# XiangFeng-Wen/STF-Unet

Hardware: AMD Instinct MI355X
Metric: training samples/sec (256x256 DCE-MRI frames) (higher is better)
Workload: dtype bf16; 1 GPU; cfg2 UNet(in=8,base_c=64) 256x256 train step; model=UNet, global_batch=64, per_gpu_batch=64, seq_len=8, parallelism=dp1, ddp_hook=False

## Files before the change

### include/stfunet.h

```cpp
#ifndef STFUNET_H
#define STFUNET_H
#include <stddef.h>
#include <stdint.h>

#ifdef __cplusplus
extern "C" {
#endif

typedef void* stf_stream_t;

typedef struct stf_conv_geom {
  int N;
  int Hs, Ws, Cs;
  int src_cstride;
  int Hd, Wd;
  int R, S;
  int stride, pad;
  int transposed;
} stf_conv_geom;

typedef struct stf_lstm_epi {
  const float* c_prev;
  float* c_out;
  void* h_out;
// ... 210 lines not shown
int stf_resize_bilinear_fwd(const float* x, int planes, int h, int w, float* y, int H, int W, stf_stream_t stream);
int stf_resize_bilinear_bwd(const float* dy, int planes, int H, int W, float* dx, int h, int w, stf_stream_t stream);
int stf_lstm_unpack_grad(const float* dwcat, const float* dbias, int C, float* dw_ih,
                         float* dw_hh, float* db_ih, float* db_hh, stf_stream_t stream);
int stf_lstm_cell_bwd(const float* gates, const float* c_t, const float* c_prev, const void* dh,
                      int dh_cstride, const float* dc_in, float* dc_out, void* dgates, int64_t M,
                      int C, stf_stream_t stream);
int stf_pk_resize(const float* x, int B, int Ttot, int T, int P, int H, int W, int h, int w,
                  void* dst, int dst_cstride, int coff, stf_stream_t stream);

int stf_eval_counts(const float* logits, const int64_t* target, int B, int K, int64_t HW,
                    int64_t ignore_index, int64_t* confmat, int64_t* dice_counts, stf_stream_t stream);
int stf_eval_counts_sm(const float* logits, const float* probs, const int64_t* target, int B, int K,
                       int64_t HW, int64_t ignore_index, int64_t* confmat, int64_t* dice_counts,
                       stf_stream_t stream);

int stf_predict_mask(const float* logits, const int64_t* target, int B, int K, int64_t HW, int rule,
                     int channel, float threshold, int64_t ignore, uint8_t* mask, int64_t* counts,
                     stf_stream_t stream);
size_t stf_predict_overlay_scratch_bytes(int B, int64_t HW);
int stf_predict_overlay(const float* frames, int64_t batch_stride, const uint8_t* mask, int B, int H,
                        int W, int c0, int c1, int c2, float alpha, int paint, uint8_t* out,
                        void* scratch, stf_stream_t stream);

int stf_tofts_forward(const float* ktrans, const float* ve, const float* vp, int P, int T,
                      const float* time_points, const float* cp_t, const float* tau,
                      const float* cp_tau, const int* n_valid, int n_conv, float dt, float* out,
                      stf_stream_t stream);
int stf_tofts_fit(const float* curves, int P, int T, const float* time_points, const float* cp_t,
                  const float* tau, const float* cp_tau, const int* n_valid, int n_conv, float dt,
                  int batch, int epochs, const float* adam_sched, float beta1, float beta2, float eps,
                  const float* bounds, float* params, stf_stream_t stream);

#define STF_AUG_HFLIP 1
#define STF_AUG_VFLIP 2
#define STF_AUG_ROTATE 4
typedef struct stf_aug_frame {
  int64_t src, rs, out;
  int H, W, H2, W2;
  int cx, cy, kx, ky;
  int oh, ow, h0, w0;
  int flags;
  int fx[6];
  int pad_;
  double m[6];
} stf_aug_frame;
int stf_augment_frames(const uint8_t* src, const stf_aug_frame* frames, int n, const int* coef,
                       uint8_t* scratch, int max_resized_px, int max_out_px, float mean, float stdv,
                       float* out, stf_stream_t stream);
int stf_augment_masks(const uint8_t* src, const stf_aug_frame* masks, int n, const int* tabs,
                      int max_out_px, int64_t* out, stf_stream_t stream);

typedef struct stf_plan stf_plan;
stf_plan* stf_plan_create(void);
void stf_plan_destroy(stf_plan* plan);
int stf_plan_record(stf_plan* plan);
int stf_plan_stop(void);
int stf_plan_size(const stf_plan* plan);
int stf_plan_tag(const char* name, double flops);
int stf_plan_tag_end(void);
int stf_plan_replay(stf_plan* plan, int first, int last, const char* timed_tag);
int stf_plan_timing(stf_plan* plan, int* launches, double* ms, double* flops);
int stf_stream_wait(stf_stream_t waiter, stf_stream_t waitee);
int stf_memset(void* p, int value, size_t bytes, stf_stream_t stream);
int stf_copy_rows(const float* src, int64_t src_ld, float* dst, int64_t dst_ld, int rows, int cols,
                  stf_stream_t stream);
int stf_i64_add_batch(int64_t* const* ptrs, int count, int64_t inc, stf_stream_t stream);

const char* stf_error_string(int code);
int stf_abi_version(void);

#define STF_STORAGE_BF16 0
#define STF_STORAGE_FP16 1
int stf_storage_type(void);

#ifdef __cplusplus
}
#endif
#endif
```

### stf-unet_amd/csrc/common.h

```cpp
#pragma once
#include <hip/hip_runtime.h>
#include <stdint.h>

#include <tuple>
#include <type_traits>
#include <utility>

#ifdef STF_FP16
typedef _Float16 e16;
#else
typedef __bf16 e16;
#endif
typedef e16 e16x8 __attribute__((ext_vector_type(8)));
typedef e16 e16x4 __attribute__((ext_vector_type(4)));
typedef short short4v __attribute__((ext_vector_type(4)));
typedef float f32x4 __attribute__((ext_vector_type(4)));
typedef float f32x16 __attribute__((ext_vector_type(16)));
typedef unsigned int u32x4v __attribute__((ext_vector_type(4)));

#define STF_DEV __device__ __forceinline__

STF_DEV float e2f(e16 v) { return (float)v; }
STF_DEV e16 f2e(float v) { return (e16)v; }

// ... 55 lines not shown
  gi = sigm(pi); gf = sigm(pf); gg = tanh_f(pg); go = sigm(po);
  c = __builtin_fmaf(gf, cp, gi * gg);
  h = go * tanh_f(c);
}
STF_DEV void lstm_cell_bwd(float gi, float gf, float gg, float go, float ct, float cp, float dh, float dcn,
                           float& d_i, float& d_f, float& d_g, float& d_o, float& dcp) {
#pragma clang fp contract(off)
  const float tc = tanh_f(ct);
  const float dct = __builtin_fmaf(dh * go, __builtin_fmaf(-tc, tc, 1.f), dcn);
  d_o = ((dh * tc) * go) * (1.f - go);
  d_i = ((dct * gg) * gi) * (1.f - gi);
  d_g = (dct * gi) * __builtin_fmaf(-gg, gg, 1.f);
  d_f = ((dct * cp) * gf) * (1.f - gf);
  dcp = dct * gf;
}

STF_DEV float wave_sum(float v) {
#pragma unroll
  for (int o = 32; o > 0; o >>= 1) v += __shfl_xor(v, o, 64);
  return v;
}

template <int CTRL>
STF_DEV float dpp_f(float v) {
  return __int_as_float(__builtin_amdgcn_update_dpp(0, __float_as_int(v), CTRL, 0xF, 0xF, true));
}

STF_DEV float row16_reduce_scatter(const float (&v)[16], int r) {
  float a[8], b[4], c[2];
  const bool h3 = r & 8, h2 = r & 4, h1 = r & 2, h0 = r & 1;
#pragma unroll
  for (int k = 0; k < 8; ++k) a[k] = (h3 ? v[k + 8] : v[k]) + dpp_f<0x140>(h3 ? v[k] : v[k + 8]);
#pragma unroll
  for (int k = 0; k < 4; ++k) b[k] = (h2 ? a[k + 4] : a[k]) + dpp_f<0x141>(h2 ? a[k] : a[k + 4]);
#pragma unroll
  for (int k = 0; k < 2; ++k) c[k] = (h1 ? b[k + 2] : b[k]) + dpp_f<0x1B>(h1 ? b[k] : b[k + 2]);
  return (h0 ? c[1] : c[0]) + dpp_f<0xB1>(h0 ? c[0] : c[1]);
}

STF_DEV double wave_sum_d(double v) {
#pragma unroll
  for (int o = 32; o > 0; o >>= 1) v += __shfl_xor(v, o, 64);
  return v;
}

namespace stf {
struct PlanOp {
  virtual ~PlanOp() {}
  virtual hipError_t run() const = 0;
};
bool plan_recording();
void plan_append(PlanOp* op, hipStream_t s);

template <class... A>
struct KernelOp final : PlanOp {
  const void* fn;
  dim3 grid, block;
  unsigned shmem;
  hipStream_t stream;
  std::tuple<A...> args;
  template <class... B>
  KernelOp(const void* f, dim3 g, dim3 b, unsigned sh, hipStream_t s, B&&... a)
      : fn(f), grid(g), block(b), shmem(sh), stream(s), args(std::forward<B>(a)...) {}
  hipError_t run() const override {
    return std::apply(
        [this](const A&... a) {
          void* p[sizeof...(A) + 1] = {const_cast<void*>(static_cast<const void*>(&a))...};
          return hipLaunchKernel(fn, grid, block, p, shmem, stream);
        },
        args);
  }
};

template <class... A, class... B>
inline void launch(void (*k)(A...), dim3 g, dim3 b, unsigned sh, hipStream_t s, B&&... args) {
  static_assert(sizeof...(A) == sizeof...(B), "kernel argument count");
  if (!plan_recording()) {
    std::tuple<std::decay_t<A>...> t(std::forward<B>(args)...);
    std::apply(
        [&](auto&... a) {
          void* p[sizeof...(A) + 1] = {static_cast<void*>(&a)...};
          (void)hipLaunchKernel((const void*)k, g, b, p, sh, s);
        },
        t);
    return;
  }
  auto* op = new KernelOp<std::decay_t<A>...>((const void*)k, g, b, sh, s, std::forward<B>(args)...);
  (void)op->run();
  plan_append(op, s);
}

hipError_t memset_async(void* p, int value, size_t bytes, hipStream_t s);
int ablation_env(const char* name);
char ab_letter(const char* name);
hipError_t memcpy_async(void* dst, const void* src, size_t bytes, hipMemcpyKind kind, hipStream_t s);
}

#undef hipLaunchKernelGGL
#define hipLaunchKernelGGL(K, G, B, SH, S, ...) ::stf::launch(K, G, B, SH, S, ##__VA_ARGS__)

#define STF_CHECK_LAUNCH() do { hipError_t e__ = hipGetLastError(); if (e__ != hipSuccess) return (int)e__; } while (0)

#define STF_EINVAL 100001
```

### stf-unet_amd/csrc/loss.hip

```cpp
#include "common.h"
#include "../../include/stfunet.h"
#include "reduce.h"

namespace {

constexpr int NT = 256;
constexpr int MAXK = 4;
constexpr int LCHUNK = 64;
constexpr float DICE_EPS = 1e-6f;

STF_DEV float lane_group_sum(float v, int CG) {
  if (CG >= 2) v += dpp_f<0xB1>(v);
  if (CG >= 4) v += dpp_f<0x4E>(v);
  if (CG >= 8) v += dpp_f<0x141>(v);
  if (CG >= 16) v += dpp_f<0x140>(v);
  for (int o = 16; o < CG; o <<= 1) v += __shfl_xor(v, o, 64);
  return v;
}

int head_tiles(long units) {
  long t = (units + NT - 1) / NT;
  return (int)(t < 1 ? 1 : (t > 1024 ? 1024 : t));
}

// ... 151 lines not shown
  __shared__ float red[NT / 64][NV];
  const int n = blockIdx.y;
  float w[K];
  if constexpr (OPT) {
#pragma unroll
    for (int k = 0; k < K; ++k) w[k] = o.cw ? o.cw[k] : 1.f;
  }
  float s[NV];
#pragma unroll
  for (int i = 0; i < NV; ++i) s[i] = 0.f;
  for (int hw = blockIdx.x * NT + threadIdx.x; hw < HW; hw += gridDim.x * NT) {
    float z[K], e[K], mx = -INFINITY;
#pragma unroll
    for (int k = 0; k < K; ++k) { z[k] = logits[((long)n * K + k) * HW + hw]; mx = fmaxf(mx, z[k]); }
    float se = 0.f;
#pragma unroll
    for (int k = 0; k < K; ++k) { e[k] = expf(z[k] - mx); se += e[k]; }
    int t = (int)target[(long)n * HW + hw];
    bool keep = true;
    if constexpr (OPT) {
      const int64_t t64 = target[(long)n * HW + hw];
      keep = !(o.ignore >= 0 && t64 == (int64_t)o.ignore);
      t = (t64 >= 0 && t64 < K) ? (int)t64 : -1;
    }
    const float inv = 1.f / se, lse = logf(se);
#pragma unroll
    for (int k = 0; k < K; ++k) {
      float p = e[k] * inv;
      if constexpr (OPT) p = keep ? p : 0.f;
      const float tk = t == k ? 1.f : 0.f;
      s[3 * k] += p * tk;
      s[3 * k + 1] += p;
      s[3 * k + 2] += tk;
      if (t == k) {
        const float nll = lse - (z[k] - mx);
        if constexpr (OPT) { s[3 * K] += w[k] * nll; s[3 * K + 1] += w[k]; }
        else s[3 * K] += nll;
      }
    }
  }
#pragma unroll
  for (int i = 0; i < NV; ++i) s[i] = wave_sum(s[i]);
  if ((threadIdx.x & 63) == 0)
#pragma unroll
    for (int i = 0; i < NV; ++i) red[threadIdx.x >> 6][i] = s[i];
  __syncthreads();
  if (threadIdx.x < NV) {
    float a = 0.f;
    for (int wv = 0; wv < NT / 64; ++wv) a += red[wv][threadIdx.x];
    part[((size_t)n * gridDim.x + blockIdx.x) * NV + threadIdx.x] = a;
  }
}

template <int K, bool OPT>
__global__ void loss_finalize_kernel(const float* __restrict__ part, int N, int hw_or_dice, float* __restrict__ terms,
                                     float* __restrict__ loss) {
  constexpr int NV = 3 * K + 1 + OPT;
  __shared__ double acc[64][NV];
  double ce = 0.0, wsum = 0.0, dsum = 0.0;
  for (int base = 0; base < N; base += 64) {
    const int n = base + (int)threadIdx.x;
    if (threadIdx.x < 64) {
      for (int i = 0; i < NV; ++i) {
        double a = 0.0;
        if (n < N)
          for (int c = 0; c < LCHUNK; ++c) a += part[((size_t)n * LCHUNK + c) * NV + i];
        acc[threadIdx.x][i] = a;
      }
    }
    __syncthreads();
    if (threadIdx.x == 0) {
      for (int r = 0; r < 64 && base + r < N; ++r) {
        for (int k = 0; k < K; ++k) {
          const double I = acc[r][3 * k], S = acc[r][3 * k + 1] + acc[r][3 * k + 2];
          const float If = (float)I, Sf = (float)S;
          const float setsum = Sf == 0.f ? 2.f * If : Sf;
          dsum += (double)((2.f * If + DICE_EPS) / (setsum + DICE_EPS));
          terms[((size_t)(base + r) * K + k) * 3 + 0] = If;
          terms[((size_t)(base + r) * K + k) * 3 + 1] = (float)acc[r][3 * k + 1];
          terms[((size_t)(base + r) * K + k) * 3 + 2] = (float)acc[r][3 * k + 2];
        }
        ce += acc[r][3 * K];
        if constexpr (OPT) wsum += acc[r][3 * K + 1];
      }
    }
    __syncthreads();
  }
  if (threadIdx.x == 0) {
    terms[(size_t)N * K * 3] = (float)ce;
    if constexpr (OPT) {
      terms[(size_t)N * K * 3 + 1] = (float)wsum;
      loss[0] = (float)(ce / wsum + (hw_or_dice ? 1.0 - dsum / ((double)N * K) : 0.0));
    } else {
      loss[0] = (float)(ce / ((double)N * hw_or_dice) + 1.0 - dsum / ((double)N * K));
    }
  }
}

template <int K, bool OPT, class... O>
__global__ void loss_bwd_kernel(const float* __restrict__ logits, const int64_t* __restrict__ target, int N, int HW,
                                const float* __restrict__ terms, const float* __restrict__ grad_out,
                                float* __restrict__ dlogits, O... opt) {
  const LossOpt<OPT> o{opt...};
  const long P = (long)N * HW;
  const float go = grad_out ? grad_out[0] : 1.f;
  float inv_den = 1.f / (float)P;
  if constexpr (OPT) inv_den = 1.f / terms[(size_t)N * K * 3 + 1];
  const float dscale = -1.f / (float)(K * N);
  float w[K];
  if constexpr (OPT) {
#pragma unroll
    for (int k = 0; k < K; ++k) w[k] = o.cw ? o.cw[k] : 1.f;
  }
  for (long i = blockIdx.x * (long)NT + threadIdx.x; i < P; i += (long)gridDim.x * NT) {
    const long n = i / HW, hw = i - n * HW;
    float z[K], mx = -INFINITY;
#pragma unroll
    for (int k = 0; k < K; ++k) { z[k] = logits[(n * K + k) * HW + hw]; mx = fmaxf(mx, z[k]); }
    float se = 0.f;
#pragma unroll
    for (int k = 0; k < K; ++k) { z[k] = expf(z[k] - mx); se += z[k]; }
    int t = (int)target[i];
    bool keep = true;
    if constexpr (OPT) {
      const int64_t t64 = target[i];
      keep = !(o.ignore >= 0 && t64 == (int64_t)o.ignore);
      t = (t64 >= 0 && t64 < K) ? (int)t64 : -1;
    }
    float p[K], G[K], pg = 0.f, wt = 0.f;
#pragma unroll
    for (int k = 0; k < K; ++k) {
      p[k] = z[k] / se;
      const float tk = t == k ? 1.f : 0.f;
      if constexpr (OPT) wt += tk * w[k];
// ... 41 lines not shown
    case 3: { constexpr int KK = 3; EXPR; } break; \
    case 4: { constexpr int KK = 4; EXPR; } break; \
    default: return STF_EINVAL;             \
  }

extern "C" int stf_head_tiles(int N, int H, int W, int C) { return head_tiles((long)N * H * W * (C / 8)); }

extern "C" int stf_head_fwd(const void* y, int N, int H, int W, int C, const float* scale, const float* shift,
                            const float* w, const float* bias, int classes, float* logits, stf_stream_t stream) {
  if (!head_ok(C)) return STF_EINVAL;
  const long P = (long)N * H * W, units = P * (C / 8);
  if (units >= (1L << 31)) return STF_EINVAL;
  long blocks = (units + NT - 1) / NT;
  if (blocks > 8192) blocks = 8192;
  hipStream_t s = (hipStream_t)stream;
  STF_KDISPATCH(classes, hipLaunchKernelGGL(head_fwd_kernel<KK>, dim3(blocks), dim3(NT), 0, s, (const uint16_t*)y,
                                            P, H * W, C, scale, shift, w, bias, logits));
  STF_CHECK_LAUNCH();
  return 0;
}

extern "C" int stf_head_bwd(const float* dlogits, const void* y, int N, int H, int W, int C, const float* scale,
                            const float* shift, const float* mean, const float* invstd, const float* w, int classes,
                            void* g_out, float* bn_partial, float* head_partial, float* dw, float* db,
                            stf_stream_t stream) {
  if (!head_ok(C) || (long)N * H * W * (C / 8) >= (1L << 31)) return STF_EINVAL;
  const long P = (long)N * H * W;
  const int tiles = stf_head_tiles(N, H, W, C);
  hipStream_t s = (hipStream_t)stream;
  STF_KDISPATCH(classes, hipLaunchKernelGGL(head_bwd_kernel<KK>, dim3(tiles), dim3(NT), 0, s, dlogits,
                                            (const uint16_t*)y, P, H * W, C, scale, shift, mean, invstd, w,
                                            (uint16_t*)g_out, bn_partial, head_partial));
  STF_CHECK_LAUNCH();
  const int HC = classes * (C + 1);
  const int S = stf::colsum_stage1(head_partial, tiles, HC, s);
  hipLaunchKernelGGL(sum_tiles_kernel, dim3((HC + 255) / 256), dim3(256), 0, s, head_partial, S, HC, classes * C,
                     dw, db);
  STF_CHECK_LAUNCH();
  return 0;
}

static int loss_scratch_floats(int N, int K, bool opt) {
  return N * K * 3 + 1 + opt + N * LCHUNK * (3 * K + 1 + opt);
}

template <bool OPT, class... O>
static int loss_fwd(const float* logits, const int64_t* target, int N, int HW, int classes, float* terms, float* loss,
                    hipStream_t s, O... opt) {
  float* part = terms + N * classes * 3 + 1 + OPT;
  const int hw_or_dice = OPT ? LossOpt<OPT>{opt...}.dice : HW;
  STF_KDISPATCH(classes, {
    hipLaunchKernelGGL((loss_fwd_kernel<KK, OPT, O...>), dim3(LCHUNK, N), dim3(NT), 0, s, logits, target, HW, part,
                       opt...);
    hipLaunchKernelGGL((loss_finalize_kernel<KK, OPT>), dim3(1), dim3(64), 0, s, part, N, hw_or_dice, terms, loss);
  });
  STF_CHECK_LAUNCH();
  return 0;
}

template <bool OPT, class... O>
static int loss_bwd(const float* logits, const int64_t* target, int N, int HW, int classes, const float* terms,
                    const float* grad_out, float* dlogits, hipStream_t s, O... opt) {
  const long P = (long)N * HW;
  long blocks = (P + NT - 1) / NT;
  if (blocks > 8192) blocks = 8192;
  STF_KDISPATCH(classes, hipLaunchKernelGGL((loss_bwd_kernel<KK, OPT, O...>), dim3(blocks), dim3(NT), 0, s, logits,
                                            target, N, HW, terms, grad_out, dlogits, opt...));
  STF_CHECK_LAUNCH();
  return 0;
}

static bool loss_opt_ok(int classes, int ignore_index) {
  return classes >= 1 && classes <= MAXK && !(ignore_index >= 0 && ignore_index < classes);
}

extern "C" int stf_loss_scratch_floats(int N, int classes) { return loss_scratch_floats(N, classes, false); }
extern "C" int stf_loss_opt_scratch_floats(int N, int classes) { return loss_scratch_floats(N, classes, true); }

extern "C" int stf_loss_fwd(const float* logits, const int64_t* target, int N, int H, int W, int classes,
                            float* terms, float* loss, stf_stream_t stream) {
  return loss_fwd<false>(logits, target, N, H * W, classes, terms, loss, (hipStream_t)stream);
}

extern "C" int stf_loss_bwd(const float* logits, const int64_t* target, int N, int H, int W, int classes,
                            const float* terms, const float* grad_out, float* dlogits, stf_stream_t stream) {
  return loss_bwd<false>(logits, target, N, H * W, classes, terms, grad_out, dlogits, (hipStream_t)stream);
}

extern "C" int stf_loss_opt_fwd(const float* logits, const int64_t* target, int N, int H, int W, int classes,
                                const float* class_weight, int ignore_index, int dice, float* terms, float* loss,
                                stf_stream_t stream) {
  if (!loss_opt_ok(classes, ignore_index)) return STF_EINVAL;
  return loss_fwd<true>(logits, target, N, H * W, classes, terms, loss, (hipStream_t)stream, class_weight,
                        ignore_index, dice);
}

extern "C" int stf_loss_opt_bwd(const float* logits, const int64_t* target, int N, int H, int W, int classes,
                                const float* class_weight, int ignore_index, int dice, const float* terms,
                                const float* grad_out, float* dlogits, stf_stream_t stream) {
  if (!loss_opt_ok(classes, ignore_index)) return STF_EINVAL;
  return loss_bwd<true>(logits, target, N, H * W, classes, terms, grad_out, dlogits, (hipStream_t)stream,
                        class_weight, ignore_index, dice);
}

namespace {

constexpr int MCK = 16;
// ... 444 lines not shown
```

### stf-unet_amd/csrc/plan.hip

```cpp
#include "common.h"
#include "../../include/stfunet.h"

#include <atomic>
#include <cstdio>
#include <cstdlib>
#include <map>
#include <memory>
#include <mutex>
#include <string>
#include <vector>

namespace {

struct TagRange {
  int first, last;
  std::string name;
  double flops;
};

}

struct stf_plan {
  std::vector<std::unique_ptr<stf::PlanOp>> ops;
  std::vector<hipStream_t> op_stream;
  std::vector<TagRange> tags;
  int open_tag = -1;
  std::vector<std::pair<hipEvent_t, hipEvent_t>> ev;
  std::vector<int> ev_range;
  size_t ev_used = 0;
  ~stf_plan() {
    for (auto& e : ev) {
      (void)hipEventDestroy(e.first);
      (void)hipEventDestroy(e.second);
    }
  }
};

namespace {

thread_local stf_plan* g_rec = nullptr;

struct MemsetOp final : stf::PlanOp {
  void* p;
  int value;
  size_t bytes;
  hipStream_t s;
  hipError_t run() const override { return hipMemsetAsync(p, value, bytes, s); }
};

struct MemcpyOp final : stf::PlanOp {
  void* dst;
  const void* src;
  size_t bytes;
  hipStream_t s;
  hipError_t run() const override { return hipMemcpyAsync(dst, src, bytes, hipMemcpyDeviceToDevice, s); }
};

struct WaitOp final : stf::PlanOp {
  hipEvent_t ev = nullptr;
  hipStream_t waiter, waitee;
  ~WaitOp() override {
    if (ev) (void)hipEventDestroy(ev);
  }
  hipError_t run() const override {
    hipError_t e = hipEventRecord(ev, waitee);
    return e != hipSuccess ? e : hipStreamWaitEvent(waiter, ev, 0);
  }
};

void append(stf::PlanOp* op, hipStream_t s) {
  g_rec->ops.emplace_back(op);
  g_rec->op_stream.push_back(s);
}

std::mutex g_pool_mu;
std::map<int, std::vector<hipEvent_t>> g_pool;
std::map<int, unsigned> g_pool_next;
constexpr int POOL = 64;

hipError_t pooled_event(hipEvent_t* out) {
  int dev = 0;
  hipError_t e = hipGetDevice(&dev);
  if (e != hipSuccess) return e;
  std::lock_guard<std::mutex> g(g_pool_mu);
  auto& v = g_pool[dev];
  if (v.size() < POOL) {
    hipEvent_t ev;
    e = hipEventCreateWithFlags(&ev, hipEventDisableTiming);
    if (e != hipSuccess) return e;
    v.push_back(ev);
    *out = ev;
    return hipSuccess;
  }
  unsigned& i = g_pool_next[dev];
  *out = v[i++ % POOL];
  return hipSuccess;
}

__global__ __launch_bounds__(256) void copy_rows_kernel(const float* __restrict__ src, int64_t src_ld,
                                                         float* __restrict__ dst, int64_t dst_ld, int rows,
                                                         int cols) {
  const int64_t n = (int64_t)rows * cols;
  for (int64_t i = (int64_t)blockIdx.x * 256 + threadIdx.x; i < n; i += (int64_t)gridDim.x * 256) {
    const int64_t r = i / cols, c = i - r * cols;
    dst[r * dst_ld + c] = src[r * src_ld + c];
  }
}

constexpr int I64_BATCH = 64;
struct I64Batch {
  int64_t* p[I64_BATCH];
};

__global__ void i64_add_kernel(I64Batch b, int n, int64_t inc) {
  if ((int)threadIdx.x < n) b.p[threadIdx.x][0] += inc;
}

}

bool stf::plan_recording() { return g_rec != nullptr; }

void stf::plan_append(stf::PlanOp* op, hipStream_t s) { append(op, s); }

int stf::ablation_env(const char* name) {
  const char* e = getenv(name);
  if (!e || !e[0] || (e[0] == '0' && !e[1])) return 0;
  const char* ok = getenv("STF_ABLATION");
  if (ok && ok[0] == '1') {
    fprintf(stderr, "stfunet: timing-only ablation %s=%s is ON -- results are not valid\n", name, e);
    return atoi(e);
  }
  fprintf(stderr, "stfunet: %s=%s ignored (a timing-only ablation: set STF_ABLATION=1 as well)\n", name, e);
  return 0;
}

char stf::ab_letter(const char* name) {
  const char* e = getenv(name);
  return e ? e[0] : 0;
}

hipError_t stf::memset_async(void* p, int value, size_t bytes, hipStream_t s) {
  if (!g_rec) return hipMemsetAsync(p, value, bytes, s);
  auto* op = new MemsetOp;
  op->p = p;
  op->value = value;
  op->bytes = bytes;
  op->s = s;
  hipError_t e = op->run();
  append(op, s);
  return e;
}

hipError_t stf::memcpy_async(void* dst, const void* src, size_t bytes, hipMemcpyKind kind, hipStream_t s) {
  if (!g_rec) return hipMemcpyAsync(dst, src, bytes, kind, s);
  if (kind != hipMemcpyDeviceToDevice) return hipErrorInvalidValue;
  auto* op = new MemcpyOp;
  op->dst = dst;
  op->src = src;
  op->bytes = bytes;
  op->s = s;
  hipError_t e = op->run();
  append(op, s);
  return e;
}

extern "C" stf_plan* stf_plan_create(void) { return new stf_plan; }

extern "C" void stf_plan_destroy(stf_plan* p) { delete p; }

extern "C" int stf_plan_record(stf_plan* p) {
  if (!p || g_rec) return STF_EINVAL;
  p->ops.clear();
  p->op_stream.clear();
  p->tags.clear();
  p->open_tag = -1;
  g_rec = p;
  return 0;
}

extern "C" int stf_plan_stop(void) {
  if (!g_rec) return STF_EINVAL;
  if (g_rec->open_tag >= 0) g_rec->tags[g_rec->open_tag].last = (int)g_rec->ops.size();
  g_rec->open_tag = -1;
  g_rec = nullptr;
  return 0;
}

extern "C" int stf_plan_size(const stf_plan* p) { return p ? (int)p->ops.size() : -1; }

extern "C" int stf_plan_tag(const char* name, double flops) {
  if (!g_rec || !name) return 0;
  stf_plan* p = g_rec;
  if (p->open_tag >= 0) p->tags[p->open_tag].last = (int)p->ops.size();
  p->tags.push_back(TagRange{(int)p->ops.size(), -1, name, flops});
  p->open_tag = (int)p->tags.size() - 1;
  return 0;
}

extern "C" int stf_plan_tag_end(void) {
  if (!g_rec || g_rec->open_tag < 0) return 0;
  g_rec->tags[g_rec->open_tag].last = (int)g_rec->ops.size();
  g_rec->open_tag = -1;
  return 0;
}

extern "C" int stf_plan_replay(stf_plan* p, int first, int last, const char* timed_tag) {
  if (!p || g_rec == p || first < 0 || last > (int)p->ops.size() || first > last) return STF_EINVAL;
  if (!timed_tag) {
    for (int i = first; i < last; ++i) {
      hipError_t e = p->ops[i]->run();
      if (e != hipSuccess) return (int)e;
    }
    return 0;
  }
  size_t r = 0;
  const size_t nr = p->tags.size();
  for (int i = first; i < last; ++i) {
    while (r < nr && (p->tags[r].first < i || p->tags[r].last <= p->tags[r].first)) ++r;
    const bool start = r < nr && p->tags[r].first == i && p->tags[r].last > i && p->tags[r].name == timed_tag;
    int stop_at = -1;
    hipStream_t ts = nullptr;
    if (start) {
      if (p->ev_used == p->ev.size()) {
        hipEvent_t a, b;
        hipError_t e = hipEventCreate(&a);
        if (e == hipSuccess) e = hipEventCreate(&b);
        if (e != hipSuccess) return (int)e;
        p->ev.emplace_back(a, b);
        p->ev_range.push_back(0);
// ... 98 lines not shown
```

### stf-unet_amd/stfunet/_lib.py

```python
import contextlib
import ctypes
import os

import torch

_HERE = os.path.dirname(os.path.abspath(__file__))
LIB_PATH = os.path.join(_HERE, "libstfunet_hip.so")
LIB_PATH = os.environ.get("STF_LIB", LIB_PATH)
LIB_PATH_F16 = os.environ.get("STF_LIB_F16", os.path.join(os.path.dirname(LIB_PATH), "libstfunet_hip_f16.so"))
LIB_PATHS = {torch.bfloat16: LIB_PATH, torch.float16: LIB_PATH_F16}
STORAGE_CODE = {torch.bfloat16: 0, torch.float16: 1}

BUILD_INFO = os.path.join(_HERE, "build_info.json")
_SRC_DIRS = (os.path.join(_HERE, "..", "csrc"), os.path.join(_HERE, "..", "..", "include"))


def _sha(paths):
    import hashlib
    h = hashlib.sha256()
    for p in paths:
        h.update(os.path.basename(p).encode())
        with open(p, "rb") as f:
            h.update(f.read())
    return h.hexdigest()[:16]
# ... 101 lines not shown
    "stf_adamw_dev": (c_int, [P, P, P, P, c_int64, P, c_float, c_float, c_float, c_float, P]),
    "stf_adamw_amp": (c_int, [P, P, P, P, c_int64, P, P, P, c_float, c_float, c_float, c_float, P]),
    "stf_pack_input": (c_int, [P, c_int, c_int, c_int, c_int, c_int, P, P]),
    "stf_pack_weight": (c_int, [P, c_int, c_int, c_int, c_int, c_int, c_int, P, P]),
    "stf_pack_weights": (c_int, [P, c_int, c_int64, P]),
    "stf_augment_frames": (c_int, [P, P, c_int, P, P, c_int, c_int, c_float, c_float, P, P]),
    "stf_augment_masks": (c_int, [P, P, c_int, P, c_int, P, P]),
    "stf_pack_tiles": (c_int, [c_int, c_int, c_int, c_int, c_int, c_int]),
    "stf_pack_weights_tiled": (c_int, [P, c_int, c_int, P]),
    "stf_pack_sequence": (c_int, [P, c_int, c_int, c_int, c_int, c_int, c_int, c_int, c_int, P, P]),
    "stf_eval_counts": (c_int, [P, P, c_int, c_int, c_int64, c_int64, P, P, P]),
    "stf_lstm_coop_sync_bytes": (c_size_t, [c_int, c_int]),
    "stf_lstm_coop_supported": (c_int, [c_int]),
    "stf_lstm_coop_fwd": (c_int, [P, P, P, c_int, c_int, c_int, P, P, c_int, P, P, c_int, c_uint, P]),
    "stf_lstm_coop_bwd": (c_int, [P, P, P, c_int, c_int, c_int, P, c_int, P, P, c_int, P, c_int, c_uint, P]),
    "stf_lstm_coop_error": (c_int, [P, c_int, c_int, P, P]),
    "stf_bilinear_ac_fwd": (c_int, [P, c_int, c_int, c_int, c_int, c_int, P, c_int, c_int, c_int, P]),
    "stf_bilinear_ac_bwd": (c_int, [P, c_int, c_int, c_int, c_int, c_int, P, c_int, c_int, c_int, P]),
    "stf_resize_bilinear_fwd": (c_int, [P, c_int, c_int, c_int, P, c_int, c_int, P]),
    "stf_resize_bilinear_bwd": (c_int, [P, c_int, c_int, c_int, P, c_int, c_int, P]),
    "stf_stat_sums": (c_int, [P, c_int, c_int, c_int, c_int, P, P]),
    "stf_bilinear_ac_bwd_tsum": (c_int, [P, c_int, c_int, c_int, c_int, c_int, c_int, P, c_int64, c_int64, c_int,
                                         c_int, P]),
    "stf_eval_counts_sm": (c_int, [P, P, P, c_int, c_int, c_int64, c_int64, P, P, P]),
    "stf_predict_mask": (c_int, [P, P, c_int, c_int, c_int64, c_int, c_int, c_float, c_int64, P, P, P]),
    "stf_predict_overlay_scratch_bytes": (c_size_t, [c_int, c_int64]),
    "stf_predict_overlay": (c_int, [P, c_int64, P, c_int, c_int, c_int, c_int, c_int, c_int, c_float, c_int, P, P,
                                    P]),
    "stf_tofts_forward": (c_int, [P, P, P, c_int, c_int, P, P, P, P, P, c_int, c_float, P, P]),
    "stf_tofts_fit": (c_int, [P, c_int, c_int, P, P, P, P, P, c_int, c_float, c_int, c_int, P, c_float, c_float,
                              c_float, P, P, P]),
    "stf_stem_im2col": (c_int, [P, c_int, c_int, c_int, c_int, c_int, c_int, c_int, c_int, c_int, c_int, c_int, P,
                                P]),
    "stf_stem_conv7_grid": (c_int, [c_int, c_int, c_int, c_int]),
    "stf_stem_conv7": (c_int, [P, c_int, c_int, c_int, c_int, c_int, P, P, P, P]),
    "stf_stem_wgrad7": (c_int, [P, c_int, c_int, c_int, c_int, c_int, P, P, P]),
    "stf_stem_dgrad7": (c_int, [P, P, c_int, c_int, c_int, c_int, c_int, c_int, P, P]),
    "stf_maxpool3s2_fwd": (c_int, [P, c_int, c_int, c_int, c_int, P, P, P]),
    "stf_maxpool3s2_bwd": (c_int, [P, P, c_int, c_int, c_int, c_int, P, P]),
    "stf_bn_act_maxpool3s2": (c_int, [P, c_int, c_int, c_int, c_int, c_int, P, P, P, P, P]),
    "stf_bn_bwd_reduce_pool3": (c_int, [P, P, P, c_int, c_int, c_int, c_int, c_int, P, P, P, P, P, P]),
    "stf_bn_bwd_apply_pool3": (c_int, [P, P, P, c_int, c_int, c_int, c_int, c_int, P, P, P, P, P]),
    "stf_lstm_pack": (c_int, [P, P, P, P, c_int, P, P, P, P]),
    "stf_lstm_unpack_grad": (c_int, [P, P, c_int, P, P, P, P, P]),
    "stf_lstm_seq_fwd": (c_int, [P, P, P, c_int, c_int, c_int, P, P, c_int, P]),
    "stf_lstm_seq_supported": (c_int, [c_int]),
    "stf_lstm_seq_bwd": (c_int, [P, P, P, P, c_int, c_int, c_int, P, P, c_int, P, P, c_int, P]),
    "stf_lstm_cell_bwd": (c_int, [P, P, P, P, c_int, P, P, P, c_int64, c_int, P]),
    "stf_pk_resize": (c_int, [P, c_int, c_int, c_int, c_int, c_int, c_int, c_int, c_int, P, c_int, c_int, P]),
    "stf_plan_create": (c_void_p, []),
    "stf_plan_destroy": (None, [P]),
    "stf_plan_record": (c_int, [P]),
    "stf_plan_stop": (c_int, []),
    "stf_plan_size": (c_int, [P]),
    "stf_plan_tag": (c_int, [ctypes.c_char_p, ctypes.c_double]),
    "stf_plan_tag_end": (c_int, []),
    "stf_plan_replay": (c_int, [P, c_int, c_int, ctypes.c_char_p]),
    "stf_plan_timing": (c_int, [P, ctypes.POINTER(c_int), ctypes.POINTER(ctypes.c_double),
                                ctypes.POINTER(ctypes.c_double)]),
    "stf_stream_wait": (c_int, [P, P]),
    "stf_memset": (c_int, [P, c_int, c_size_t, P]),
    "stf_copy_rows": (c_int, [P, c_int64, P, c_int64, c_int, c_int, P]),
    "stf_i64_add_batch": (c_int, [ctypes.POINTER(c_void_p), c_int, c_int64, P]),
    "stf_error_string": (ctypes.c_char_p, [c_int]),
    "stf_abi_version": (c_int, []),
    "stf_storage_type": (c_int, []),
}

EXPORTED = tuple(_SIGS)
_libs = {}
_active = torch.bfloat16
_FNS = {}
_FN = _FNS.setdefault(_active, {})


def load(dtype=None):
    dtype = _active if dtype is None else dtype
    lib = _libs.get(dtype)
    if lib is not None:
        return lib
    if dtype not in LIB_PATHS:
        raise ValueError(f"no stfunet library for storage dtype {dtype} (bf16 or fp16)")
    path = LIB_PATHS[dtype]
    if not os.path.exists(path):
        raise RuntimeError(f"stfunet HIP library not built ({path}); run `make -C stf-unet_amd/csrc` "
                           "or __graft_entry__.build()")
    lib = ctypes.CDLL(path)
    for name, (res, args) in _SIGS.items():
        fn = getattr(lib, name)
        fn.restype = res
        fn.argtypes = args
    if lib.stf_storage_type() != STORAGE_CODE[dtype]:
        raise RuntimeError(f"{path} was built for another storage type ({lib.stf_storage_type()})")
    _libs[dtype] = lib
    return lib


def storage_dtype():
    return _active


def storage_for(requested=None):
    if requested is not None:
        return requested
    if torch.is_autocast_enabled("cuda") and torch.get_autocast_dtype("cuda") == torch.float16:
        return torch.float16
# ... 46 lines not shown
```

### stf-unet_amd/stfunet/plan.py

```python
import contextlib
import ctypes
import gc
import os
import threading
import weakref
from collections import OrderedDict

import torch

from . import _lib, nhwc
from ._lib import call

TIMED = None
RECORD_HOOK = None

_POOL_LOCK = threading.RLock()
_POOL_ACTIVE = 0
_GRAVEYARD = []


POOL_EVENTS = {"buried": 0, "destroyed": 0, "entry_del": 0}


def _bury(pool):
    if pool is not None:
        with _POOL_LOCK:
            _GRAVEYARD.append(pool)
            POOL_EVENTS["buried"] += 1


def drain_pools():
    with _POOL_LOCK:
        if _POOL_ACTIVE or not _GRAVEYARD:
            return
        dead = _GRAVEYARD[:]
        _GRAVEYARD.clear()
        POOL_EVENTS["destroyed"] += len(dead)
        dead.clear()


@contextlib.contextmanager
def _pool_context(pool):
    global _POOL_ACTIVE
    if pool is None:
        yield
        return
    with _POOL_LOCK:
        _POOL_ACTIVE += 1
    try:
        with torch.cuda.use_mem_pool(pool):
            yield
    finally:
        with _POOL_LOCK:
            _POOL_ACTIVE -= 1
        drain_pools()


def _stf_env():
    data = getattr(os.environ, "_data", None)
    if isinstance(data, dict):
        return tuple(sorted((k, v) for k, v in data.items() if k.startswith(b"STF_")))
    return tuple(sorted((k, v) for k, v in os.environ.items() if k.startswith("STF_")))


def enabled():
    return os.environ.get("STF_PLAN", "1") != "0" and not torch.cuda.is_current_stream_capturing()


class Plan:

    def __init__(self):
        self.lib = _lib.load()
        self.h = self.lib.stf_plan_create()
        if not self.h:
            raise MemoryError("stf_plan_create failed")
        self.n = 0

    def record(self, fn):
        _lib.check(self.lib.stf_plan_record(self.h), "stf_plan_record")
        nhwc.RECORDING = True
        try:
            return fn()
        finally:
            nhwc.RECORDING = False
            _lib.check(self.lib.stf_plan_stop(), "stf_plan_stop")
            self.n = self.lib.stf_plan_size(self.h)

    def size(self):
        return self.lib.stf_plan_size(self.h)

    def replay(self, first=0, last=None):
        last = self.n if last is None else last
        if last > first:
            tag = TIMED.encode() if TIMED is not None else None
            _lib.check(self.lib.stf_plan_replay(self.h, first, last, tag), "stf_plan_replay")

    def timing(self):
        n, ms, fl = ctypes.c_int(0), ctypes.c_double(0.0), ctypes.c_double(0.0)
        _lib.check(self.lib.stf_plan_timing(self.h, ctypes.byref(n), ctypes.byref(ms), ctypes.byref(fl)),
                   "stf_plan_timing")
        return n.value, ms.value, fl.value

    def __del__(self):
        h, self.h = getattr(self, "h", None), None
        if h:
            self.lib.stf_plan_destroy(h)


@contextlib.contextmanager
def _no_gc():
    was = gc.isenabled()
    gc.disable()
    try:
        yield
    finally:
        if was:
            gc.enable()


def _new_pool():
    if os.environ.get("STF_PLAN_POOL", "1") == "0" or not hasattr(torch.cuda, "MemPool"):
        return None
    return torch.cuda.MemPool()


class _Entry:

    def __init__(self):
        self.seen = 0
        self.fwd = self.bwd = None
        self.x = self.logits = self.S = None
        self.bsig = None
        self.dl = None
        self.marks = []
        self.keep = []
        self.bkeep = []
        self.pool = None
        self.owner = None

    def release(self):
        pool, self.pool = self.pool, None
        self.fwd = self.bwd = None
        self.x = self.logits = self.S = self.dl = None
        self.keep, self.bkeep = [], []
        _bury(pool)

    def __del__(self):
        POOL_EVENTS["entry_del"] += 1
        pool = getattr(self, "pool", None)
        if pool is not None:
            self.pool = None
            _bury(pool)

    def busy(self):
        o = self.owner() if self.owner is not None else None
        return o is not None and self.S is not None and getattr(o, "saved", None) is self.S


class StepRuntime:

    def __init__(self, prog):
        self._prog = weakref.ref(prog)
        self._bns = None
        self.warm = int(os.environ.get("STF_PLAN_WARM", "1"))
        self.slots = max(1, int(os.environ.get("STF_PLAN_SLOTS", "2")))
        self._bufs = None
        self.entries = OrderedDict()
        self.cur = None

    @property
    def prog(self):
        p = self._prog()
        if p is None:
            raise RuntimeError("StepRuntime: its program is gone")
        return p

    def close(self):
        for e in self.entries.values():
            e.release()
        self.entries.clear()
        self.cur = None
        drain_pools()

    @property
    def fwd(self):
        return self.cur.fwd if self.cur is not None else None

    @property
    def bwd(self):
        return self.cur.bwd if self.cur is not None else None

    def _signature(self, x, training):
        p = self.prog
        if self._bufs is None:
            self._bufs = [(mod, n) for mod in p.m.modules() for n in mod._buffers
                          if mod._buffers[n] is not None]
            self._bufd = ([mod._buffers for mod, _ in self._bufs], [n for _, n in self._bufs])
            self._bns = [mod for mod in p.m.modules() if isinstance(mod, torch.nn.modules.batchnorm._BatchNorm)]
        bufs = tuple(map(torch.Tensor.data_ptr, map(dict.__getitem__, *self._bufd)))
        bn = tuple((b.momentum, b.eps) for b in self._bns)
        env = _stf_env()
        knobs = p.plan_knobs() if hasattr(p, "plan_knobs") else ()
        return (tuple(x.shape), x.dtype, x.device, training, _lib.storage_dtype(), _lib.stream(),
                p.flat.data.data_ptr(), bufs, bn, env, knobs)

    def _entry(self, sig):
        e = self.entries.get(sig)
        if e is None:
            while len(self.entries) >= self.slots:
                _, old = self.entries.popitem(last=False)
                if old is self.cur:
                    self.cur = None
                old.release()
            e = self.entries[sig] = _Entry()
        else:
            self.entries.move_to_end(sig)
        return e

    def forward(self, x, training, need_bwd, ctx=None):
        p = self.prog
        drain_pools()
        if not (enabled() and training and need_bwd and nhwc.TIMER is None):
            return p.forward(x, training, need_bwd)
        e = self._entry(self._signature(x, training))
        if e.busy():
            return p.forward(x, training, need_bwd)
        if e.fwd is None:
            e.seen += 1
            if e.seen <= self.warm:
                return p.forward(x, training, need_bwd)
            self._record_forward(e, x, training)
        else:
            e.x.copy_(x)
            e.fwd.replay()
        if ctx is not None:
            e.owner = weakref.ref(ctx)
        self.cur = e
        return e.logits, e.S

    def own(self, S, ctx):
        e = self.cur
        if e is not None and S is not None and e.S is S:
            e.owner = weakref.ref(ctx)

    def _record_forward(self, e, x, training):
        with _no_gc():
            self._record_forward_pooled(e, x, training)

    def _record_forward_pooled(self, e, x, training):
        e.pool = _new_pool()
        nhwc.KEEP = e.keep
        prog = self.prog

        def run():
            if RECORD_HOOK is not None:
                RECORD_HOOK(self, "forward")
            return prog.forward(e.x, training, True)
        try:
            with _pool_context(e.pool):
                e.x = nhwc.empty(tuple(x.shape), x.dtype, x.device)
                e.x.copy_(x)
                plan = Plan()
                e.logits, e.S = plan.record(run)
        finally:
            nhwc.KEEP = None
        e.fwd = plan

    def backward(self, S, dlogits):
        p = self.prog
        e = next((v for v in self.entries.values() if v.fwd is not None and v.S is S), None)
        if e is None or not enabled() or nhwc.TIMER is not None:
            return p.backward(S, dlogits)
        bsig = (tuple(dlogits.shape), p.flat.grad.data_ptr(), p.grad_ready_hook is not None, _lib.stream())
        if e.bwd is None or bsig != e.bsig:
            return self._record_backward(e, S, dlogits, bsig)
        e.dl.copy_(dlogits)
        pos = 0
        hook = p.grad_ready_hook
        for idx, off, deps in e.marks:
            e.bwd.replay(pos, idx)
            hook(off, deps)
            pos = idx
        e.bwd.replay(pos)

    def _record_backward(self, e, S, dlogits, bsig):
        with _no_gc():
            self._record_backward_pooled(e, S, dlogits, bsig)

    def _record_backward_pooled(self, e, S, dlogits, bsig):
        p = self.prog
        e.bwd = None
        e.bkeep = []
        nhwc.KEEP = e.bkeep
        plan = Plan()
        marks = []
        real_hook = p.grad_ready_hook
        pend = []
        if real_hook is not None:
            def hook(off, deps=()):
                pend.extend(d for d in deps if all(d is not q for q in pend))
                acted = real_hook(off, deps)
                if acted is None or acted:
                    marks.append((plan.size(), off, tuple(pend)))
                    pend.clear()
            p.grad_ready_hook = hook

        def run():
            if RECORD_HOOK is not None:
                RECORD_HOOK(self, "backward")
            return p.backward(S, e.dl)
        try:
            with _pool_context(e.pool):
                e.dl = nhwc.empty(tuple(dlogits.shape), dlogits.dtype, dlogits.device)
                e.dl.copy_(dlogits)
                plan.record(run)
        finally:
            nhwc.KEEP = None
            p.grad_ready_hook = real_hook
        e.bwd, e.bsig, e.marks = plan, bsig, marks

    def timing(self):
        tot = [0, 0.0, 0.0]
        for e in self.entries.values():
            for pl in (e.fwd, e.bwd):
                if pl is not None:
                    n, ms, fl = pl.timing()
                    tot[0] += n
                    tot[1] += ms
                    tot[2] += fl
        return tuple(tot)
```

Baseline: 2787 samples/s.

## Bind recorded plans to caller input buffers and parallelize loss finalize

Adds extern-buffer slots to recorded launch plans: during recording, kernel pointer arguments that fall inside the input or dlogits buffers are noted, so at replay the plan can be repointed at the caller's tensors instead of copying them into static buffers. This removes the per-step device copies of x and dlogits, at the cost of pointer-patching bookkeeping and a fallback whenever pointers sit inside opaque structs. Separately, the loss finalize kernel now runs 512 threads that stage per-chunk partials through shared memory with coalesced loads, instead of 64 threads doing strided serial sums.

```diff
diff --git a/include/stfunet.h b/include/stfunet.h
--- a/include/stfunet.h
+++ b/include/stfunet.h
@@ -286,6 +286,9 @@
                       int max_out_px, int64_t* out, stf_stream_t stream);
 
 typedef struct stf_plan stf_plan;
+int stf_plan_extern(stf_plan* plan, int slot, const void* base, size_t bytes);
+int stf_plan_extern_refs(const stf_plan* plan, int slot);
+int stf_plan_bind(stf_plan* plan, int slot, const void* ptr);
 stf_plan* stf_plan_create(void);
 void stf_plan_destroy(stf_plan* plan);
 int stf_plan_record(stf_plan* plan);
diff --git a/stf-unet_amd/csrc/common.h b/stf-unet_amd/csrc/common.h
--- a/stf-unet_amd/csrc/common.h
+++ b/stf-unet_amd/csrc/common.h
@@ -131,6 +131,16 @@
 bool plan_recording();
 void plan_append(PlanOp* op, hipStream_t s);
 
+bool plan_has_extern();
+void plan_note_ptr(void* loc);
+void plan_note_blob(const void* p, size_t bytes);
+
+template <class T>
+inline void plan_note_arg(T& a) {
+  if constexpr (std::is_pointer_v<T>) plan_note_ptr((void*)&a);
+  else if constexpr (std::is_class_v<T> && sizeof(T) >= sizeof(void*)) plan_note_blob(&a, sizeof(T));
+}
+
 template <class... A>
 struct KernelOp final : PlanOp {
   const void* fn;
@@ -165,6 +175,7 @@
     return;
   }
   auto* op = new KernelOp<std::decay_t<A>...>((const void*)k, g, b, sh, s, std::forward<B>(args)...);
+  if (plan_has_extern()) std::apply([](auto&... a) { (plan_note_arg(a), ...); }, op->args);
   (void)op->run();
   plan_append(op, s);
 }
diff --git a/stf-unet_amd/csrc/loss.hip b/stf-unet_amd/csrc/loss.hip
--- a/stf-unet_amd/csrc/loss.hip
+++ b/stf-unet_amd/csrc/loss.hip
@@ -227,34 +227,59 @@
   }
 }
 
+constexpr int FIN_NT = 512;
+static_assert(LCHUNK == 64, "the finalize stages one image's chunks with one lane per chunk");
 template <int K, bool OPT>
-__global__ void loss_finalize_kernel(const float* __restrict__ part, int N, int hw_or_dice, float* __restrict__ terms,
-                                     float* __restrict__ loss) {
-  constexpr int NV = 3 * K + 1 + OPT;
+__global__ __launch_bounds__(FIN_NT) void loss_finalize_kernel(const float* __restrict__ part, int N, int hw_or_dice,
+                                                               float* __restrict__ terms, float* __restrict__ loss) {
+  constexpr int NV = 3 * K + 1 + OPT, NW = FIN_NT / 64;
+  __shared__ float stage[NW][LCHUNK * NV];
   __shared__ double acc[64][NV];
+  __shared__ double dk[64][K];
+  const int lane = threadIdx.x & 63, wv = threadIdx.x >> 6;
   double ce = 0.0, wsum = 0.0, dsum = 0.0;
   for (int base = 0; base < N; base += 64) {
-    const int n = base + (int)threadIdx.x;
-    if (threadIdx.x < 64) {
-      for (int i = 0; i < NV; ++i) {
+    const int rows = N - base < 64 ? N - base : 64;
+    float v[NV];
+    if (wv < rows) {
+      const float* src = part + (size_t)(base + wv) * (LCHUNK * NV);
+#pragma unroll
+      for (int j = 0; j < NV; ++j) v[j] = src[j * 64 + lane];
+    }
+    for (int r0 = 0; r0 < rows; r0 += NW) {
+      const int r = r0 + wv;
+      if (r < rows) {
+#pragma unroll
+        for (int j = 0; j < NV; ++j) stage[wv][j * 64 + lane] = v[j];
+      }
+      __syncthreads();
+      if (r + NW < rows) {
+        const float* src = part + (size_t)(base + r + NW) * (LCHUNK * NV);
+#pragma unroll
+        for (int j = 0; j < NV; ++j) v[j] = src[j * 64 + lane];
+      }
+      if (r < rows && lane < NV) {
         double a = 0.0;
-        if (n < N)
-          for (int c = 0; c < LCHUNK; ++c) a += part[((size_t)n * LCHUNK + c) * NV + i];
-        acc[threadIdx.x][i] = a;
-      }
+#pragma unroll 8
+        for (int c = 0; c < LCHUNK; ++c) a += stage[wv][c * NV + lane];
+        acc[r][lane] = a;
+      }
+      __syncthreads();
+    }
+    for (int e = threadIdx.x; e < rows * K; e += FIN_NT) {
+      const int r = e / K, k = e - r * K;
+      const double I = acc[r][3 * k], S = acc[r][3 * k + 1] + acc[r][3 * k + 2];
+      const float If = (float)I, Sf = (float)S;
+      const float setsum = Sf == 0.f ? 2.f * If : Sf;
+      dk[r][k] = (double)((2.f * If + DICE_EPS) / (setsum + DICE_EPS));
+      terms[((size_t)(base + r) * K + k) * 3 + 0] = If;
+      terms[((size_t)(base + r) * K + k) * 3 + 1] = (float)acc[r][3 * k + 1];
+      terms[((size_t)(base + r) * K + k) * 3 + 2] = (float)acc[r][3 * k + 2];
     }
     __syncthreads();
     if (threadIdx.x == 0) {
-      for (int r = 0; r < 64 && base + r < N; ++r) {
-        for (int k = 0; k < K; ++k) {
-          const double I = acc[r][3 * k], S = acc[r][3 * k + 1] + acc[r][3 * k + 2];
-          const float If = (float)I, Sf = (float)S;
-          const float setsum = Sf == 0.f ? 2.f * If : Sf;
-          dsum += (double)((2.f * If + DICE_EPS) / (setsum + DICE_EPS));
-          terms[((size_t)(base + r) * K + k) * 3 + 0] = If;
-          terms[((size_t)(base + r) * K + k) * 3 + 1] = (float)acc[r][3 * k + 1];
-          terms[((size_t)(base + r) * K + k) * 3 + 2] = (float)acc[r][3 * k + 2];
-        }
+      for (int r = 0; r < rows; ++r) {
+        for (int k = 0; k < K; ++k) dsum += dk[r][k];
         ce += acc[r][3 * K];
         if constexpr (OPT) wsum += acc[r][3 * K + 1];
       }
@@ -402,7 +427,8 @@
   STF_KDISPATCH(classes, {
     hipLaunchKernelGGL((loss_fwd_kernel<KK, OPT, O...>), dim3(LCHUNK, N), dim3(NT), 0, s, logits, target, HW, part,
                        opt...);
-    hipLaunchKernelGGL((loss_finalize_kernel<KK, OPT>), dim3(1), dim3(64), 0, s, part, N, hw_or_dice, terms, loss);
+    hipLaunchKernelGGL((loss_finalize_kernel<KK, OPT>), dim3(1), dim3(FIN_NT), 0, s, part, N, hw_or_dice, terms,
+                       loss);
   });
   STF_CHECK_LAUNCH();
   return 0;
diff --git a/stf-unet_amd/csrc/plan.hip b/stf-unet_amd/csrc/plan.hip
--- a/stf-unet_amd/csrc/plan.hip
+++ b/stf-unet_amd/csrc/plan.hip
@@ -4,6 +4,7 @@
 #include <atomic>
 #include <cstdio>
 #include <cstdlib>
+#include <cstring>
 #include <map>
 #include <memory>
 #include <mutex>
@@ -16,6 +17,17 @@
   int first, last;
   std::string name;
   double flops;
+};
+
+struct ExtBuf {
+  uintptr_t base;
+  size_t bytes;
+  int slot;
+};
+struct ExtPatch {
+  void** loc;
+  int slot;
+  ptrdiff_t delta;
 };
 
 }
@@ -28,6 +40,9 @@
   std::vector<std::pair<hipEvent_t, hipEvent_t>> ev;
   std::vector<int> ev_range;
   size_t ev_used = 0;
+  std::vector<ExtBuf> ext;
+  std::vector<ExtPatch> patches;
+  bool ext_opaque = false;
   ~stf_plan() {
     for (auto& e : ev) {
       (void)hipEventDestroy(e.first);
@@ -67,6 +82,12 @@
     return e != hipSuccess ? e : hipStreamWaitEvent(waiter, ev, 0);
   }
 };
+
+const ExtBuf* ext_of(uintptr_t v) {
+  for (const ExtBuf& b : g_rec->ext)
+    if (v >= b.base && v - b.base < b.bytes) return &b;
+  return nullptr;
+}
 
 void append(stf::PlanOp* op, hipStream_t s) {
   g_rec->ops.emplace_back(op);
@@ -122,6 +143,25 @@
 
 void stf::plan_append(stf::PlanOp* op, hipStream_t s) { append(op, s); }
 
+bool stf::plan_has_extern() { return g_rec && !g_rec->ext.empty(); }
+
+void stf::plan_note_ptr(void* loc) {
+  if (!g_rec || g_rec->ext.empty()) return;
+  uintptr_t v;
+  memcpy(&v, loc, sizeof v);
+  if (const ExtBuf* b = ext_of(v))
+    g_rec->patches.push_back(ExtPatch{(void**)loc, b->slot, (ptrdiff_t)(v - b->base)});
+}
+
+void stf::plan_note_blob(const void* p, size_t bytes) {
+  if (!g_rec || g_rec->ext.empty()) return;
+  for (size_t o = 0; o + sizeof(uintptr_t) <= bytes; o += 4) {
+    uintptr_t v;
+    memcpy(&v, (const char*)p + o, sizeof v);
+    if (ext_of(v)) g_rec->ext_opaque = true;
+  }
+}
+
 int stf::ablation_env(const char* name) {
   const char* e = getenv(name);
   if (!e || !e[0] || (e[0] == '0' && !e[1])) return 0;
@@ -146,6 +186,7 @@
   op->value = value;
   op->bytes = bytes;
   op->s = s;
+  stf::plan_note_ptr(&op->p);
   hipError_t e = op->run();
   append(op, s);
   return e;
@@ -159,6 +200,8 @@
   op->src = src;
   op->bytes = bytes;
   op->s = s;
+  stf::plan_note_ptr(&op->dst);
+  stf::plan_note_ptr((void*)&op->src);
   hipError_t e = op->run();
   append(op, s);
   return e;
@@ -174,7 +217,33 @@
   p->op_stream.clear();
   p->tags.clear();
   p->open_tag = -1;
+  p->ext.clear();
+  p->patches.clear();
+  p->ext_opaque = false;
   g_rec = p;
+  return 0;
+}
+
+extern "C" int stf_plan_extern(stf_plan* p, int slot, const void* base, size_t bytes) {
+  if (!p || g_rec != p || slot < 0 || !base || !bytes) return STF_EINVAL;
+  for (const ExtBuf& b : p->ext)
+    if (b.slot == slot) return STF_EINVAL;
+  p->ext.push_back(ExtBuf{(uintptr_t)base, bytes, slot});
+  return 0;
+}
+
+extern "C" int stf_plan_extern_refs(const stf_plan* p, int slot) {
+  if (!p) return -1;
+  if (p->ext_opaque) return -1;
+  int n = 0;
+  for (const ExtPatch& q : p->patches) n += q.slot == slot;
+  return n;
+}
+
+extern "C" int stf_plan_bind(stf_plan* p, int slot, const void* ptr) {
+  if (!p || g_rec == p || !ptr || ((uintptr_t)ptr & 15)) return STF_EINVAL;
+  for (const ExtPatch& q : p->patches)
+    if (q.slot == slot) *q.loc = (char*)const_cast<void*>(ptr) + q.delta;
   return 0;
 }
 
diff --git a/stf-unet_amd/stfunet/_lib.py b/stf-unet_amd/stfunet/_lib.py
--- a/stf-unet_amd/stfunet/_lib.py
+++ b/stf-unet_amd/stfunet/_lib.py
@@ -177,6 +177,9 @@
     "stf_plan_destroy": (None, [P]),
     "stf_plan_record": (c_int, [P]),
     "stf_plan_stop": (c_int, []),
+    "stf_plan_extern": (c_int, [P, c_int, P, c_size_t]),
+    "stf_plan_extern_refs": (c_int, [P, c_int]),
+    "stf_plan_bind": (c_int, [P, c_int, P]),
     "stf_plan_size": (c_int, [P]),
     "stf_plan_tag": (c_int, [ctypes.c_char_p, ctypes.c_double]),
     "stf_plan_tag_end": (c_int, []),
diff --git a/stf-unet_amd/stfunet/plan.py b/stf-unet_amd/stfunet/plan.py
--- a/stf-unet_amd/stfunet/plan.py
+++ b/stf-unet_amd/stfunet/plan.py
@@ -75,16 +75,30 @@
         if not self.h:
             raise MemoryError("stf_plan_create failed")
         self.n = 0
-
-    def record(self, fn):
+        self.refs = {}
+        self.at = {}
+        self.bound = 0
+        self.copied = 0
+
+    def record(self, fn, extern=()):
         _lib.check(self.lib.stf_plan_record(self.h), "stf_plan_record")
         nhwc.RECORDING = True
         try:
+            for slot, t in extern:
+                _lib.check(self.lib.stf_plan_extern(self.h, slot, t.data_ptr(), t.numel() * t.element_size()),
+                           "stf_plan_extern")
             return fn()
         finally:
             nhwc.RECORDING = False
             _lib.check(self.lib.stf_plan_stop(), "stf_plan_stop")
             self.n = self.lib.stf_plan_size(self.h)
+            self.refs = {slot: self.lib.stf_plan_extern_refs(self.h, slot) for slot, _ in extern}
+            self.at = {slot: t.data_ptr() for slot, t in extern}
+
+    def bind(self, slot, ptr):
+        if self.at.get(slot) != ptr:
+            _lib.check(self.lib.stf_plan_bind(self.h, slot, ptr), "stf_plan_bind")
+            self.at[slot] = ptr
 
     def size(self):
         return self.lib.stf_plan_size(self.h)
@@ -105,6 +119,14 @@
         h, self.h = getattr(self, "h", None), None
         if h:
             self.lib.stf_plan_destroy(h)
+
+
+X_SLOT, DL_SLOT = 0, 1
+
+
+def _in_place(t, static):
+    return (t.dtype == static.dtype and t.device == static.device and t.shape == static.shape
+            and t.is_contiguous() and t.data_ptr() % 16 == 0)
 
 
 @contextlib.contextmanager
@@ -130,6 +152,7 @@
         self.seen = 0
         self.fwd = self.bwd = None
         self.x = self.logits = self.S = None
+        self.xsrc = None
         self.bsig = None
         self.dl = None
         self.marks = []
@@ -141,7 +164,7 @@
     def release(self):
         pool, self.pool = self.pool, None
         self.fwd = self.bwd = None
-        self.x = self.logits = self.S = self.dl = None
+        self.x = self.logits = self.S = self.dl = self.xsrc = None
         self.keep, self.bkeep = [], []
         _bury(pool)
 
@@ -231,7 +254,16 @@
                 return p.forward(x, training, need_bwd)
             self._record_forward(e, x, training)
         else:
-            e.x.copy_(x)
+            if (e.fwd.refs.get(X_SLOT, 0) > 0 and (e.bwd is None or e.bwd.refs.get(X_SLOT, 0) >= 0)
+                    and _in_place(x, e.x)):
+                e.xsrc = x
+                e.fwd.bind(X_SLOT, x.data_ptr())
+                e.fwd.bound += 1
+            else:
+                e.xsrc = None
+                e.x.copy_(x)
+                e.fwd.bind(X_SLOT, e.x.data_ptr())
+                e.fwd.copied += 1
             e.fwd.replay()
         if ctx is not None:
             e.owner = weakref.ref(ctx)
@@ -260,8 +292,9 @@
             with _pool_context(e.pool):
                 e.x = nhwc.empty(tuple(x.shape), x.dtype, x.device)
                 e.x.copy_(x)
+                e.xsrc = None
                 plan = Plan()
-                e.logits, e.S = plan.record(run)
+                e.logits, e.S = plan.record(run, extern=((X_SLOT, e.x),))
         finally:
             nhwc.KEEP = None
         e.fwd = plan
@@ -274,7 +307,15 @@
         bsig = (tuple(dlogits.shape), p.flat.grad.data_ptr(), p.grad_ready_hook is not None, _lib.stream())
         if e.bwd is None or bsig != e.bsig:
             return self._record_backward(e, S, dlogits, bsig)
-        e.dl.copy_(dlogits)
+        if e.bwd.refs.get(DL_SLOT, 0) > 0 and _in_place(dlogits, e.dl):
+            e.bwd.bind(DL_SLOT, dlogits.data_ptr())
+            e.bwd.bound += 1
+        else:
+            e.dl.copy_(dlogits)
+            e.bwd.bind(DL_SLOT, e.dl.data_ptr())
+            e.bwd.copied += 1
+        if e.bwd.refs.get(X_SLOT, 0) > 0:
+            e.bwd.bind(X_SLOT, (e.xsrc if e.xsrc is not None else e.x).data_ptr())
         pos = 0
         hook = p.grad_ready_hook
         for idx, off, deps in e.marks:
@@ -313,7 +354,9 @@
             with _pool_context(e.pool):
                 e.dl = nhwc.empty(tuple(dlogits.shape), dlogits.dtype, dlogits.device)
                 e.dl.copy_(dlogits)
-                plan.record(run)
+                if e.xsrc is not None:
+                    e.x.copy_(e.xsrc)
+                plan.record(run, extern=((X_SLOT, e.x), (DL_SLOT, e.dl)))
         finally:
             nhwc.KEEP = None
             p.grad_ready_hook = real_hook
```

After: 2783 samples/s (median of 2 runs). Within noise of the previous version (-0.1%).
